# Ignalina/znippy

Measured on NVIDIA B200. Metric: decode+blake3-verify GB/s (device), higher is better.
Workload: dtype u8/u32

## Files before the change

znippy_b200/csrc/blake3_kernels.cuh:

```cuda
#pragma once
#include "blake3.cuh"
#include "xxh_verify.cuh"

namespace zn {

ZN_D const uint8_t* content_ptr(const BlobDesc& d, const uint8_t* blobs_base, const uint8_t* out_base) {
  return (d.flags & F_COMPRESSED) ? out_base + d.dst_off : blobs_base + d.src_off;
}

constexpr int kB3Warps = 8;
constexpr int kB3RowBytes = 128;
constexpr int kB3RowStride = kB3RowBytes + 16;
constexpr int kB3Stages = 2;
constexpr int kB3StageBytes = 32 * kB3RowStride;
constexpr int kB3SmemPerWarp = kB3Stages * kB3StageBytes;
constexpr int kB3RowsPerIssue = 32 / (kB3RowBytes / 16);

ZN_D void cp_async16(void* smem_dst, const void* gmem_src) {
  const uint32_t s = (uint32_t)__cvta_generic_to_shared(smem_dst);
  asm volatile("cp.async.cg.shared.global [%0], [%1], 16;\n" ::"r"(s), "l"(gmem_src) : "memory");
}
ZN_D void cp_async_commit() { asm volatile("cp.async.commit_group;\n" ::: "memory"); }
template <int N>
ZN_D void cp_async_wait() { asm volatile("cp.async.wait_group %0;\n" ::"n"(N) : "memory"); }
// ... 87 lines not shown

__global__ void __launch_bounds__(kB3Warps * 32) k_b3_chunks(const BlobDesc* __restrict__ blobs,
                                                              const uint32_t* __restrict__ chunk_prefix,
                                                              uint32_t n_blobs, uint32_t chunk_lo, uint32_t chunk_hi,
                                                              const uint8_t* __restrict__ blobs_base,
                                                              const uint8_t* __restrict__ out_base,
                                                              uint32_t* cvs, uint32_t one) {
  extern __shared__ __align__(16) uint8_t b3_smem[];
  const uint32_t lane = threadIdx.x & 31u, warp = threadIdx.x >> 5;
  uint8_t* wbuf = b3_smem + warp * kB3SmemPerWarp;
  const uint32_t n_tiles = (chunk_hi - chunk_lo + 31u) >> 5;
  const uint32_t warps_total = gridDim.x * kB3Warps;
  for (uint32_t tile = blockIdx.x * kB3Warps + warp; tile < n_tiles; tile += warps_total) {
    const uint32_t g = chunk_lo + tile * 32u + lane;
    const bool act = g < chunk_hi;
    const uint8_t* ptr = nullptr;
    uint32_t len = 0, ctr = 0;
    bool root = false, skip = false;
    if (act) {
      uint32_t lo = 0, hi = n_blobs;
      while (hi - lo > 1) {
        const uint32_t mid = (lo + hi) >> 1;
        if (__ldg(chunk_prefix + mid) <= g) lo = mid; else hi = mid;
      }
      const BlobDesc d = blobs[lo];
      skip = (d.flags & F_HASHED) != 0;
      ctr = g - __ldg(chunk_prefix + lo);
      ptr = content_ptr(d, blobs_base, out_base) + (uint64_t)ctr * kChunk;
      const uint64_t remain = d.dst_cap - (uint64_t)ctr * kChunk;
      len = remain < kChunk ? (uint32_t)remain : kChunk;
      root = d.n_chunks == 1;
    }
    if (__all_sync(0xFFFFFFFFu, !act || skip)) continue;
    uint32_t cv[8];
    b3_warp_tile(wbuf, ptr, len, ctr, root, act && !skip, lane, one, cv);
    if (act && !skip) b3::store_cv(cvs + (uint64_t)g * 8, cv);
  }
}

ZN_D void finish_blob(const BlobDesc& d, uint32_t blob, const uint32_t (&cv)[8], uint32_t* __restrict__ digests,
                      const uint32_t* __restrict__ expect, uint32_t* __restrict__ status, const uint8_t* blobs_base,
                      const uint8_t* out_base) {
  b3::store_cv(digests + (uint64_t)blob * 8, cv);
  if (out_base && status[blob] == S_OK && xxh_row_bad(d, blobs_base, out_base)) status[blob] = S_DECODE_ERROR;
  if ((d.flags & F_HAS_EXPECT) && status[blob] == S_OK) {
    bool eq = true;
#pragma unroll
    for (int i = 0; i < 8; i++) eq &= (__ldg(expect + (uint64_t)blob * 8 + i) == cv[i]);
    if (!eq) status[blob] = S_DIGEST_MISMATCH;
  }
}

__global__ void __launch_bounds__(128) k_b3_tree_small(const BlobDesc* __restrict__ blobs,
                                                       const uint32_t* __restrict__ list, uint32_t n_list,
                                                       uint32_t* cvs, uint32_t* __restrict__ digests,
                                                       const uint32_t* __restrict__ expect,
                                                       uint32_t* __restrict__ status, uint32_t one,
                                                       const uint8_t* blobs_base, const uint8_t* out_base) {
  const uint32_t t = blockIdx.x * blockDim.x + threadIdx.x;
  if (t >= n_list) return;
  const uint32_t blob = list[t];
  const BlobDesc d = blobs[blob];
  uint32_t* base = cvs + d.cv_base * 8;
  uint32_t n = d.n_chunks;
  uint32_t l[8], r[8], o[8];
  while (n > 1) {
    const uint32_t pairs = n >> 1;
    for (uint32_t j = 0; j < pairs; j++) {
      b3::load_cv(base + (uint64_t)(2 * j) * 8, l);
      b3::load_cv(base + (uint64_t)(2 * j + 1) * 8, r);
      b3::parent(l, r, n == 2, o, one);
      b3::store_cv(base + (uint64_t)j * 8, o);
    }
    if (n & 1) {
      b3::load_cv(base + (uint64_t)(n - 1) * 8, l);
      b3::store_cv(base + (uint64_t)pairs * 8, l);
    }
    n = pairs + (n & 1);
  }
  b3::load_cv(base, o);
  finish_blob(d, blob, o, digests, expect, status, blobs_base, out_base);
}

__global__ void __launch_bounds__(512) k_b3_tree_large(const BlobDesc* __restrict__ blobs,
                                                       const uint32_t* __restrict__ list,
                                                       uint32_t* cvs, uint32_t* cvs2, uint32_t* __restrict__ digests,
                                                       const uint32_t* __restrict__ expect,
                                                       uint32_t* __restrict__ status, uint32_t one,
                                                       const uint8_t* blobs_base, const uint8_t* out_base) {
  const uint32_t blob = list[blockIdx.x];
  const BlobDesc d = blobs[blob];
  uint32_t* src = cvs + d.cv_base * 8;
  uint32_t* dst = cvs2 + d.cv_base * 8;
  uint32_t n = d.n_chunks;
  uint32_t l[8], r[8], o[8];
  while (n > 1) {
    const uint32_t pairs = n >> 1, items = pairs + (n & 1);
    for (uint32_t j = threadIdx.x; j < items; j += blockDim.x) {
      b3::load_cv(src + (uint64_t)(2 * j) * 8, l);
      if (j < pairs) {
        b3::load_cv(src + (uint64_t)(2 * j + 1) * 8, r);
        b3::parent(l, r, n == 2, o, one);
      } else {
#pragma unroll
        for (int i = 0; i < 8; i++) o[i] = l[i];
      }
      b3::store_cv(dst + (uint64_t)j * 8, o);
    }
    __syncthreads();
    uint32_t* t = src; src = dst; dst = t;
    n = items;
  }
  if (threadIdx.x == 0) {
    b3::load_cv(src, o);
    finish_blob(d, blob, o, digests, expect, status, blobs_base, out_base);
  }
}

constexpr uint32_t kTreeSmallMax = 64;

}
```

znippy_b200/csrc/fused_ws.cuh:

```cuda
#pragma once
#include "blake3_kernels.cuh"
#include "decode_kernels.cuh"

namespace zn {

constexpr int kWsTeamThreads = 128;
constexpr int kWsTeams = 2;
constexpr int kWsTeamWarps = kWsTeamThreads / 32;
constexpr int kWsDecWarps = kWsTeams * kWsTeamWarps;
constexpr int kWsHashWarps = 16;
constexpr int kWsThreads = 32 * (kWsDecWarps + kWsHashWarps);
constexpr uint32_t kWsTileBytes = 32u * kChunk;

struct WsDecRegion {
  alignas(128) uint8_t tile[kTileBytes];
  alignas(16) uint8_t src[kSrcStage + 32];
  DecShared sh;
  uint32_t base;
};

constexpr uint32_t kWsTeamBytes =
    ((sizeof(WsDecRegion) > (size_t)kWsTeamWarps * kB3SmemPerWarp ? sizeof(WsDecRegion) : (size_t)kWsTeamWarps * kB3SmemPerWarp) + 127u) & ~127u;
constexpr uint32_t kWsSmemBytes = kWsTeams * kWsTeamBytes + kWsHashWarps * kB3SmemPerWarp;
static_assert(kWsSmemBytes <= 227u * 1024u, "one CTA per SM");

struct WsQueue {
  uint32_t* ctl;
  unsigned long long* ent;
  uint32_t total;
};

#ifdef ZN_WS_DEBUG
__device__ unsigned long long g_ws_dbg[4];
ZN_D unsigned long long ws_now() { unsigned long long t; asm volatile("mov.u64 %0, %%globaltimer;" : "=l"(t)); return t; }
#endif

ZN_D void ws_push(const WsQueue& q, uint32_t list_idx, uint32_t first_tile, uint32_t count) {
  if (!count) return;
  __threadfence();
  const uint32_t pos = atomicAdd(q.ctl + 1, count);
  for (uint32_t i = 0; i < count; i++)
    *reinterpret_cast<volatile unsigned long long*>(q.ent + pos + i) = ((unsigned long long)list_idx << 32) | (first_tile + i + 1u);
}

struct WsHook {
  WsQueue q;
  uint32_t list_idx, cap, pushed;
  ZN_D void after_block(const Team& t, zs::ExecState& es) {
    if (es.pos - es.wm >= (1u << 20)) zs::mem_sync(t, es);
    const uint32_t w = es.wm < cap ? es.wm : cap;
    const uint32_t ready = w / kWsTileBytes;
    if (t.tid == t.n - 1u && ready > pushed) ws_push(q, list_idx, pushed, ready - pushed);
    if (ready > pushed) pushed = ready;
  }
  ZN_D void finish(const Team&, zs::ExecState&) {}
};

__global__ void __launch_bounds__(kWsThreads, 1)
    k_decode_ws(const BlobDesc* __restrict__ blobs, const uint32_t* __restrict__ list, uint32_t n_list, const uint8_t* blobs_base,
                uint8_t* out_base, uint8_t* lit_scratch, uint32_t* status, uint32_t* produced, uint32_t* work_counter, uint32_t* cvs,
                WsQueue q, uint32_t one) {
  extern __shared__ __align__(128) uint8_t ws_smem[];
  const uint32_t warp = threadIdx.x >> 5, lane = threadIdx.x & 31u;
#ifdef ZN_WS_DEBUG
  if (threadIdx.x == 0) atomicMin(&g_ws_dbg[0], ws_now());
#endif

  if (warp < (uint32_t)kWsDecWarps) {
    const uint32_t team = warp / kWsTeamWarps;
    WsDecRegion* dr = reinterpret_cast<WsDecRegion*>(ws_smem + team * kWsTeamBytes);
    const Team t{threadIdx.x - team * kWsTeamThreads, (uint32_t)kWsTeamThreads, 1u + team};
    DecShared* sh = &dr->sh;
    if (t.tid == 0) sh->tile = dr->tile;
    zs::init_luts(t, sh);
    uint8_t* lit = lit_scratch + (size_t)(blockIdx.x * kWsTeams + team) * kLitStride;
    uint32_t predef = 0;
    for (;;) {
      if (t.tid == 0) dr->base = atomicAdd(work_counter, 1u);
      team_sync(t);
      const uint32_t base = dr->base;
      if (base >= n_list) break;
      const uint32_t blob = list[base];
      const BlobDesc d = blobs[blob];
      WsHook hook{q, base, (uint32_t)d.dst_cap, 0u};
      uint32_t st, got = 0;
      if (d.src_len >= 0xFFFFFFF0ull || d.dst_cap >= 0xFFFFFFF0ull) {
        st = S_UNSUPPORTED;
      } else {
        const uint8_t* src = blobs_base + d.src_off;
        if (d.src_len <= kSrcStage) {
          team_copy(t, dr->src + 16, src, (uint32_t)d.src_len);
          team_sync(t);
          src = dr->src + 16;
        }
        if (d.flags & F_LZ4_BLOCK) {
          st = decode_lz4_block(t, sh, src, (uint32_t)d.src_len, out_base + d.dst_off, (uint32_t)d.dst_cap, &got);
        } else {
          st = decode_blob(t, sh, src, (uint32_t)d.src_len, out_base + d.dst_off, (uint32_t)d.dst_cap, lit, predef, &got, hook);
        }
        if (st == S_OK && got != (uint32_t)d.dst_cap) st = S_SIZE_MISMATCH;
      }
      if (t.tid < kBulkIssuers) bulk_wait_all();
      team_sync(t);
      if (t.tid == 0) {
        status[blob] = st;
        produced[blob] = got;
      }
      if (t.tid == t.n - 1u) {
        const uint32_t n_tiles = (d.n_chunks + 31u) / 32u;
        ws_push(q, base, hook.pushed, n_tiles - hook.pushed);
      }
    }
#ifdef ZN_WS_DEBUG
    if (t.tid == 0) { atomicMax(&g_ws_dbg[1], ws_now()); atomicMax(&g_ws_dbg[3], (unsigned long long)*(volatile uint32_t*)q.ctl); }
#endif
    team_sync(t);
  }

  uint8_t* wbuf = warp < (uint32_t)kWsDecWarps
                      ? ws_smem + (warp / kWsTeamWarps) * kWsTeamBytes + (warp % kWsTeamWarps) * kB3SmemPerWarp
                      : ws_smem + kWsTeams * kWsTeamBytes + (warp - kWsDecWarps) * kB3SmemPerWarp;
  for (;;) {
    uint32_t idx = 0, e_lo = 0, e_hi = 0;
    if (lane == 0) {
      idx = atomicAdd(q.ctl, 1u);
      if (idx < q.total) {
        unsigned long long e;
        uint32_t spins = 0;
        while ((e = *reinterpret_cast<volatile unsigned long long*>(q.ent + idx)) == 0ull) {
          __nanosleep(100);
          if (++spins > (1u << 25) || ((spins & 4095u) == 0 && *reinterpret_cast<volatile uint32_t*>(q.ctl + 2))) {
            atomicExch(q.ctl + 2, 1u);
            idx = 0xFFFFFFFFu;
            break;
          }
        }
        __threadfence();
        e_lo = (uint32_t)e;
        e_hi = (uint32_t)(e >> 32);
      }
    }
    idx = __shfl_sync(0xFFFFFFFFu, idx, 0);
    if (idx >= q.total) break;
    const uint32_t tile = __shfl_sync(0xFFFFFFFFu, e_lo, 0) - 1u, li = __shfl_sync(0xFFFFFFFFu, e_hi, 0);
    const BlobDesc d = blobs[list[li]];
    const uint32_t cap = (uint32_t)d.dst_cap;
    const uint32_t g = tile * 32u + lane;
    const bool act = g < d.n_chunks;
    const uint32_t rem = act ? cap - min(cap, g * kChunk) : 0u;
    uint32_t cv[8];
#ifdef ZN_WS_NOHASH
    for (int k = 0; k < 8; k++) cv[k] = 0;
#else
    b3_warp_tile(wbuf, out_base + d.dst_off + (size_t)g * kChunk, rem < kChunk ? rem : kChunk, g, d.n_chunks == 1, act, lane, one, cv);
#endif
    if (act) b3::store_cv(cvs + (size_t)d.cv_base * 8 + (size_t)g * 8, cv);
  }
#ifdef ZN_WS_DEBUG
  if (lane == 0) atomicMax(&g_ws_dbg[2], ws_now());
#endif
}

}
```

znippy_b200/csrc/znippy_cuda.cu:

```cuda
#include <cuda_runtime.h>

#include <algorithm>
#include <chrono>
#include <cstdio>
#include <cstring>
#include <mutex>
#include <numeric>
#include <string>
#include <unordered_map>
#include <vector>

#define ZN_BACKBITS_DEPTH 1
#include "../../include/znippy_cuda.h"
#include "blake3_kernels.cuh"
#include "host_api.h"
#include "decode_kernels.cuh"
#include "par_kernel.cuh"
#include "fused_ws.cuh"

using namespace zn;

struct zn_ctx {
  int device = 0;
  int sm_count = 0;
  cudaStream_t stream = nullptr;
  cudaStream_t stream2 = nullptr;
  void* pinned = nullptr;
  size_t pinned_bytes = 0;
  uint8_t* plan_pin = nullptr;
  size_t plan_pin_cap = 0, plan_pin_used = 0;
  template <typename T>
  T* arena(size_t count) {
    plan_pin_used = (plan_pin_used + 63) & ~(size_t)63;
    T* r = reinterpret_cast<T*>(plan_pin + plan_pin_used);
    plan_pin_used += count * sizeof(T);
    return r;
  }
  uint8_t* d_lit = nullptr;
  uint8_t* d_par = nullptr;
  uint32_t dec_grid = 0;
  uint32_t dec_grid_small = 0;
  uint8_t* d_in = nullptr;
  size_t d_in_cap = 0;
  uint8_t* d_out = nullptr;
  size_t d_out_cap = 0;
  CompressScratch cs;
  struct ZScratch {
    zp::ZBlock* blocks = nullptr; uint32_t* comp_list = nullptr; size_t slots = 0;
    zp::FseD* tabs = nullptr; size_t tab_sets = 0;
    zp::SeqRec16* recs = nullptr; size_t seqs = 0;
    zp::SeqP1* p1 = nullptr; size_t p1s = 0;
    uint8_t* lits = nullptr; size_t lit16 = 0;
    zp::ZPools* pools = nullptr;
  } zs;
  uint64_t launches = 0;
  std::string err;
};

enum PlanKind { PLAN_DECODE_VERIFY = 1, PLAN_HASH = 2, PLAN_COMPRESS = 3 };

enum DecClass {
  DC_PIPE = 0,
  DC_BIGPAT,
  DC_BIGRAW,
  DC_SMALL,
  DC_MID,
  DC_COUNT
};

struct zn_plan {
  zn_ctx* ctx = nullptr;
  int kind = 0;
  uint32_t n = 0;
  uint32_t total_chunks = 0;
  uint32_t n_dec = 0, n_small = 0, n_large = 0, n_pieces = 0;
  BlobDesc* d_blobs = nullptr;
  uint32_t* d_chunk_prefix = nullptr;
  uint32_t *d_list_dec = nullptr, *d_list_small = nullptr, *d_list_large = nullptr;
  uint32_t *d_piece_blob = nullptr, *d_piece_idx = nullptr;
  uint64_t* d_magic_off = nullptr;
  uint32_t n_magic = 0;
  uint32_t *d_cvs = nullptr, *d_digests = nullptr, *d_expect = nullptr, *d_status = nullptr, *d_produced = nullptr,
           *d_counter = nullptr, *d_wsq = nullptr, *d_cvs2 = nullptr, *d_status0 = nullptr;
  uint32_t ws_tiles = 0;
  bool ran_ws = false;
  cudaEvent_t ev[4] = {nullptr, nullptr, nullptr, nullptr};
  cudaStream_t last_stream = nullptr;
  bool ran = false;
  uint32_t cls_off[DC_COUNT + 1] = {0};
  uint32_t n_hashed = 0;
  zp::ZBlob* d_zb = nullptr;
  uint32_t nzb = 0;
  size_t z_slots = 0, z_tabs = 0, z_seqs = 0, z_lit16 = 0;
  uint64_t z_mean = 0;
  bool uploads_synced = false;
  uint32_t launches_per_run = 0;
  CompressScratch cs;
  CompressPrep cp;
  zn_plan* hp = nullptr;
  bool envelope = false;
  uint64_t capacity = 0;
  std::vector<uint32_t> h_status;
};

static const int kDecodeThreads = 128;
static const int kDecodeCtasPerSm = 4;

#define ZN_CUDA(ctx, call)                                                              \
  do {                                                                                  \
    cudaError_t e__ = (call);                                                           \
    if (e__ != cudaSuccess) {                                                           \
      (ctx)->err = std::string(#call) + ": " + cudaGetErrorString(e__);                 \
      return ZN_E_CUDA;                                                                 \
    }                                                                                   \
  } while (0)

extern "C" int zn_abi_version(void) { return ZN_ABI_VERSION; }

extern "C" int zn_device_count(void) {
  int n = 0;
  if (cudaGetDeviceCount(&n) != cudaSuccess) return 0;
  return n;
}

extern "C" const char* zn_strerror(int code) {
  switch (code) {
    case ZN_OK: return "ok";
    case ZN_E_ARG: return "invalid argument";
    case ZN_E_CUDA: return "CUDA error";
    case ZN_E_NOMEM: return "out of memory";
    case ZN_E_STATE: return "call out of order";
    default: return "unknown error";
  }
}

extern "C" const char* zn_status_name(uint32_t s) {
  switch (s) {
    case ZN_S_OK: return "OK";
    case ZN_S_DECODE_ERROR: return "DECODE_ERROR";
    case ZN_S_DIGEST_MISMATCH: return "DIGEST_MISMATCH";
    case ZN_S_DST_TOO_SMALL: return "DST_TOO_SMALL";
    case ZN_S_UNSUPPORTED: return "UNSUPPORTED";
    case ZN_S_SIZE_MISMATCH: return "SIZE_MISMATCH";
    default: return "?";
  }
}

static void build_predef(PredefTables* p) {
  static zs::FseTable t;
  uint16_t next[64];
  zs::fse_build(&t, zs::kLLDefault, 36, 6, next);
  for (int i = 0; i < 64; i++) p->ll[i] = t.e[i];
  zs::fse_build(&t, zs::kOFDefault, 29, 5, next);
  for (int i = 0; i < 32; i++) p->of[i] = t.e[i];
  zs::fse_build(&t, zs::kMLDefault, 53, 6, next);
  for (int i = 0; i < 64; i++) p->ml[i] = t.e[i];
}

extern "C" zn_ctx* zn_ctx_create(int device, size_t staging_bytes) {
  int ndev = 0;
  if (cudaGetDeviceCount(&ndev) != cudaSuccess || device < 0 || device >= ndev) return nullptr;
  if (cudaSetDevice(device) != cudaSuccess) return nullptr;
  zn_ctx* c = new zn_ctx();
  c->device = device;
  cudaDeviceProp prop;
  if (cudaGetDeviceProperties(&prop, device) != cudaSuccess) { delete c; return nullptr; }
// ... 164 lines not shown
    BlobDesc& d = descs[i];
    const bool comp = kind == PLAN_DECODE_VERIFY && compressed && compressed[i];
    d.src_off = src_off[i];
    d.src_len = src_len[i];
    if (comp && compressed[i] == 3) {
      if (d.src_off < 4) { delete p; c->err = "compressed == 3 needs four bytes in front of the payload"; return nullptr; }
      d.src_off -= 4;
      d.src_len += 4;
      magic_off.push_back(d.src_off);
    }
    d.dst_off = out_off ? out_off[i] : 0;
    d.dst_cap = kind == PLAN_DECODE_VERIFY ? (out_len ? out_len[i] : 0) : src_len[i];
    bool skip = false;
    if (!comp && kind == PLAN_DECODE_VERIFY && d.dst_cap != d.src_len) {
      status0[i] = S_SIZE_MISMATCH;
      any_status = true;
      skip = true;
      d.src_len = 0;
      d.dst_cap = 0;
    }
    const uint64_t nc = std::max<uint64_t>(1, (d.dst_cap + kChunk - 1) / kChunk);
    d.n_chunks = (uint32_t)nc;
    d.cv_base = chunks;
    d.flags = (comp ? F_COMPRESSED : 0u) | (expect && !skip ? F_HAS_EXPECT : 0u) | (comp && compressed[i] == 2 ? F_LZ4_BLOCK : 0u);
    prefix[i] = (uint32_t)chunks;
    chunks += nc;
    if (chunks > 0xFFFFFFF0ull) { delete p; c->err = "batch too large (chunk count)"; return nullptr; }
    if (comp) {
      const bool big = d.dst_cap >= (512u << 10), pat = d.src_len * 64 <= d.dst_cap, lz4b = (d.flags & F_LZ4_BLOCK) != 0;
      int k;
      if (big && pat && !lz4b) k = DC_BIGPAT;
      else if (!lz4b && !pat && d.src_len < d.dst_cap && d.dst_cap >= 4096 && d.dst_cap < 0xFFFFFFF0ull) k = DC_PIPE;
      else if (big) k = DC_BIGRAW;
      else if (d.dst_cap <= (64u << 10)) k = DC_SMALL;
      else k = DC_MID;
      cls[k].push_back(i);
    } else if (gather_raw && kind == PLAN_DECODE_VERIFY && !skip)
      for (uint64_t o = 0, k = 0; o < d.dst_cap; o += kGatherPiece, k++) { pblob.push_back(i); pidx.push_back((uint32_t)k); }
    if (nc <= kTreeSmallMax) lsmall_a[n_lsmall++] = i; else llarge.push_back(i);
  }
  prefix[n] = (uint32_t)chunks;
  p->total_chunks = (uint32_t)chunks;
  uint32_t* ldec = c->arena<uint32_t>(n);
  uint32_t n_ldec = 0;
  for (int k = 0; k < DC_COUNT; k++) {
    auto& L = cls[k];
    bool sorted_desc = true;
    for (size_t j = 1; j < L.size() && sorted_desc; j++) sorted_desc = descs[L[j]].dst_cap <= descs[L[j - 1]].dst_cap;
    if (!sorted_desc) std::stable_sort(L.begin(), L.end(), [&](uint32_t x, uint32_t y) { return descs[x].dst_cap > descs[y].dst_cap; });
    p->cls_off[k] = n_ldec;
    if (!L.empty()) memcpy(ldec + n_ldec, L.data(), L.size() * 4);
    n_ldec += (uint32_t)L.size();
  }
  p->cls_off[DC_COUNT] = n_ldec;
  p->n_dec = n_ldec;
  for (uint32_t i : cls[DC_BIGPAT]) { descs[i].flags |= F_HASHED; p->ws_tiles += (descs[i].n_chunks + 31u) / 32u; p->n_hashed++; }
  std::vector<zp::ZBlob> zb(cls[DC_PIPE].size());
  {
    uint64_t slots = 0, seqs = 0, lit16 = 0, tabs = 0, bytes = 0;
    for (size_t j = 0; j < zb.size(); j++) {
      const uint64_t cap = descs[cls[DC_PIPE][j]].dst_cap;
      const uint32_t sc = (uint32_t)(cap / 16384 + 8);
      memset(&zb[j], 0, sizeof zb[j]);
      zb[j].blob = cls[DC_PIPE][j];
      zb[j].slot0 = (uint32_t)slots;
      zb[j].slot_cap = sc;
      slots += sc;
      seqs += cap / 5 + 64;
      lit16 += cap / 16 + 2ull * sc + 2;
      tabs += cap / 32768 + 2;
      bytes += cap;
    }
    const uint64_t lim = 0xFFFFFFF0ull;
    p->nzb = (uint32_t)zb.size();
    p->z_slots = (size_t)std::min(slots, lim);
    p->z_seqs = (size_t)std::min(seqs, lim);
    p->z_lit16 = (size_t)std::min(lit16, lim);
    p->z_tabs = (size_t)std::min(tabs, lim);
    p->z_mean = zb.empty() ? 0 : bytes / zb.size();
    if (slots > lim) { delete p; c->err = "batch too large (zstd block slots)"; return nullptr; }
  }
  p->n_small = n_lsmall;
  p->n_large = (uint32_t)llarge.size();
  p->n_pieces = (uint32_t)pblob.size();
  p->n_magic = (uint32_t)magic_off.size();
  bool ok = upload(c, &p->d_blobs, descs, n) && upload(c, &p->d_chunk_prefix, prefix, (size_t)n + 1) &&
            upload(c, &p->d_list_dec, ldec, n_ldec) && upload(c, &p->d_list_small, lsmall_a, n_lsmall) &&
            upload(c, &p->d_list_large, llarge.data(), llarge.size()) &&
            upload(c, &p->d_piece_blob, pblob.data(), pblob.size()) && upload(c, &p->d_piece_idx, pidx.data(), pidx.size()) &&
            upload(c, &p->d_magic_off, magic_off.data(), magic_off.size()) &&
            upload(c, &p->d_expect, (const uint32_t*)expect, expect ? (size_t)n * 8 : 0) &&
            upload(c, &p->d_cvs, (const uint32_t*)nullptr, (size_t)chunks * 8) &&
            upload(c, &p->d_cvs2, (const uint32_t*)nullptr, llarge.empty() ? 0 : (size_t)chunks * 8) &&
            upload(c, &p->d_digests, (const uint32_t*)nullptr, (size_t)n * 8) &&
            upload(c, &p->d_status, (const uint32_t*)nullptr, n) && upload(c, &p->d_produced, (const uint32_t*)nullptr, n) &&
            upload(c, &p->d_counter, (const uint32_t*)nullptr, 16) &&
            upload(c, &p->d_wsq, (const uint32_t*)nullptr, cls[DC_BIGPAT].empty() ? 0 : 6 + 2 * (size_t)p->ws_tiles) &&
            upload(c, &p->d_zb, zb.data(), zb.size());
  if (ok && any_status) ok = upload(c, &p->d_status0, status0, n);
  for (int i = 0; ok && i < 4; i++) ok = cudaEventCreate(&p->ev[i]) == cudaSuccess;
  if (ok) ok = cudaStreamSynchronize(c->stream) == cudaSuccess;
  if (!ok) {
    c->err = std::string("plan allocation failed: ") + cudaGetErrorString(cudaGetLastError());
    zn_plan_destroy(p);
    return nullptr;
  }
  p->uploads_synced = true;
  return p;
}

extern "C" zn_plan* zn_plan_decode_verify(zn_ctx* ctx, uint32_t n, const uint64_t* h_blob_off, const uint64_t* h_blob_len,
                                          const uint8_t* h_compressed, const uint64_t* h_out_off,
                                          const uint64_t* h_out_len, const uint8_t* h_expect_digest) {
  if (n && (!h_out_len || !h_compressed)) return nullptr;
  return plan_build(ctx, PLAN_DECODE_VERIFY, n, h_blob_off, h_blob_len, h_compressed, h_out_off, h_out_len,
                    h_expect_digest, h_out_off != nullptr);
}

extern "C" zn_plan* zn_plan_hash(zn_ctx* ctx, uint32_t n, const uint64_t* h_off, const uint64_t* h_len,
                                 const uint8_t* h_expect_digest) {
  return plan_build(ctx, PLAN_HASH, n, h_off, h_len, nullptr, nullptr, nullptr, h_expect_digest, false);
}

extern "C" int zn_plan_fused(const zn_plan* p) { return p && p->cls_off[DC_BIGPAT + 1] > p->cls_off[DC_BIGPAT] ? 1 : 0; }

extern "C" int zn_plan_class_counts(const zn_plan* p, uint32_t counts[5]) {
  if (!p || !counts) return ZN_E_ARG;
  if (p->kind == PLAN_COMPRESS) return ZN_E_STATE;
  for (int k = 0; k < DC_COUNT; k++) counts[k] = p->cls_off[k + 1] - p->cls_off[k];
  return ZN_OK;
}

extern "C" int zn_plan_pipeline_fallbacks(zn_plan* p, uint32_t* rows) {
  if (!p || !rows) return ZN_E_ARG;
  if (p->kind == PLAN_COMPRESS) return ZN_E_STATE;
  *rows = 0;
  if (!p->nzb || !p->ran) return ZN_OK;
  cudaSetDevice(p->ctx->device);
  if (cudaStreamSynchronize(p->last_stream) != cudaSuccess) { p->ctx->err = cudaGetErrorString(cudaGetLastError()); return ZN_E_CUDA; }
  std::vector<zp::ZBlob> hz(p->nzb);
  if (cudaMemcpy(hz.data(), p->d_zb, sizeof(zp::ZBlob) * p->nzb, cudaMemcpyDeviceToHost) != cudaSuccess) { p->ctx->err = cudaGetErrorString(cudaGetLastError()); return ZN_E_CUDA; }
  for (auto& b : hz) *rows += b.state != 0;
  return ZN_OK;
}

extern "C" void zn_plan_destroy(zn_plan* p) {
  if (!p) return;
  cudaSetDevice(p->ctx->device);
  if (p->ran) cudaStreamSynchronize(p->last_stream);
  void* ptrs[] = {p->d_blobs, p->d_chunk_prefix, p->d_list_dec, p->d_list_small, p->d_list_large, p->d_piece_blob,
                  p->d_piece_idx, p->d_cvs, p->d_digests, p->d_expect, p->d_status, p->d_produced, p->d_counter, p->d_wsq, p->d_cvs2,
                  p->d_zb, p->d_status0, p->d_magic_off};
  for (void* q : ptrs)
    if (q) cudaFreeAsync(q, p->ctx->stream);
  for (auto& e : p->ev)
    if (e) cudaEventDestroy(e);
  if (p->hp) zn_plan_destroy(p->hp);
  p->cs.release();
  delete p;
}

template <typename T>
static bool zgrow(T** ptr, size_t* have, size_t want, size_t bytes_per) {
  if (*have >= want) return true;
  if (*ptr) cudaFree(*ptr);
  *ptr = nullptr;
  *have = 0;
  const size_t cap = want + want / 8 + 16;
  if (cudaMalloc((void**)ptr, cap * bytes_per) != cudaSuccess) { cudaGetLastError(); return false; }
  *have = cap;
  return true;
}

static int run_pipeline(zn_plan* p, const uint8_t* d_blobs, uint8_t* d_out, cudaStream_t st, uint32_t* launches) {
  zn_ctx* c = p->ctx;
  auto& z = c->zs;
  if (!z.pools && cudaMalloc((void**)&z.pools, sizeof(zp::ZPools)) != cudaSuccess) { c->err = "zstd pipeline scratch allocation failed"; cudaGetLastError(); return ZN_E_NOMEM; }
  {
    const size_t slots_before = z.slots;
    size_t dummy = slots_before;
    if (!zgrow(&z.blocks, &z.slots, p->z_slots, sizeof(zp::ZBlock)) || !zgrow(&z.comp_list, &dummy, p->z_slots, 4) ||
        !zgrow(&z.tabs, &z.tab_sets, p->z_tabs, sizeof(zp::FseD) * zp::kTabSet) || !zgrow(&z.recs, &z.seqs, p->z_seqs, sizeof(zp::SeqRec16)) || !zgrow(&z.p1, &z.p1s, p->z_seqs, sizeof(zp::SeqP1)) ||
        !zgrow(&z.lits, &z.lit16, p->z_lit16 + 4, 16)) {
      c->err = "zstd pipeline scratch allocation failed";
      return ZN_E_NOMEM;
    }
  }
  zp::ZArgs a;
  a.blobs = p->d_blobs; a.blobs_base = d_blobs; a.zb = p->d_zb; a.nzb = p->nzb; a.blocks = z.blocks; a.pools = z.pools;
  a.comp_list = z.comp_list; a.tabs = z.tabs; a.recs = z.recs; a.lits = z.lits; a.p1 = z.p1;
  const bool prof = getenv("ZN_ZPROF") != nullptr;
  cudaEvent_t pe[9];
  if (prof) for (auto& e : pe) cudaEventCreate(&e);
  uint32_t* ctr = p->d_counter + DC_COUNT;
  zp::PipelineLaunch L;
  L.a = a;
  L.slots = (uint32_t)p->z_slots; L.seq_cap = (uint32_t)p->z_seqs; L.lit_cap16 = (uint32_t)p->z_lit16; L.tab_cap = (uint32_t)p->z_tabs;
  L.sm_count = (uint32_t)c->sm_count;
  L.mean_bytes = p->z_mean;
  L.d_out = d_out; L.produced = p->d_produced; L.exec_counter = ctr;
  const uint32_t pipe_launches = zp::pipeline_enqueue(L, st, prof ? pe : nullptr);
  const uint32_t* list = p->d_list_dec + p->cls_off[DC_PIPE];
  const uint32_t grid = std::min<uint32_t>(p->nzb, c->dec_grid);
  k_decode<kDecodeThreads, 1><<<grid, kDecodeThreads, 0, st>>>(p->d_blobs, list, p->nzb, d_blobs, d_out, c->d_lit, p->d_status,
                                                            p->d_produced, ctr + 1, nullptr, 1u, &p->d_zb[0].state,
                                                            (uint32_t)(sizeof(zp::ZBlob) / 4));
  if (prof) {
    cudaEventRecord(pe[7], st);
    cudaEventSynchronize(pe[7]);
    static const char* names[] = {"walk", "tables", "seq", "lit", "chain", "exec", "legacy"};
    zp::ZPools hp;
    cudaMemcpy(&hp, z.pools, sizeof hp, cudaMemcpyDeviceToHost);
    std::vector<zp::ZBlob> hz(p->nzb);
    cudaMemcpy(hz.data(), p->d_zb, sizeof(zp::ZBlob) * p->nzb, cudaMemcpyDeviceToHost);
    uint32_t handed = 0;
    for (auto& b : hz) handed += b.state != 0;
    fprintf(stderr, "zpipe: %u blobs (%u handed back), %u blocks, %u seqs, %u table sets, %u lit16 |", p->nzb, handed, hp.comp_used, hp.seq_used, hp.tab_used, hp.lit_used16);
    for (int i = 0; i < 7; i++) { float ms = 0; cudaEventElapsedTime(&ms, pe[i], pe[i + 1]); fprintf(stderr, " %s %.3f", names[i], ms); }
    if (getenv("ZN_ZPROF_SEQ1")) { float ms = 0; if (cudaEventElapsedTime(&ms, pe[2], pe[8]) == cudaSuccess) fprintf(stderr, " (seq phase 1 %.3f)", ms); else cudaGetLastError(); }
    fprintf(stderr, " ms\n");
    zp::pipeline_trace_dump();
    for (auto& e : pe) cudaEventDestroy(e);
  }
  *launches += pipe_launches + 1;
  return ZN_OK;
}

extern "C" int zn_plan_run(zn_plan* p, const uint8_t* d_blobs, uint8_t* d_out, void* stream_v) {
  if (!p) return ZN_E_ARG;
  if (p->kind == PLAN_COMPRESS) return ZN_E_STATE;
  zn_ctx* c = p->ctx;
  cudaSetDevice(c->device);
  cudaStream_t st = stream_v ? (cudaStream_t)stream_v : c->stream;
  if (p->n && !d_blobs) return ZN_E_ARG;
  if (p->n_dec && !d_out) return ZN_E_ARG;
  if (st != c->stream && !p->uploads_synced) {
    ZN_CUDA(c, cudaStreamSynchronize(c->stream));
    p->uploads_synced = true;
  }
  uint32_t launches = 0;
  ZN_CUDA(c, cudaEventRecord(p->ev[0], st));
  if (p->n) {
    if (p->d_status0) ZN_CUDA(c, cudaMemcpyAsync(p->d_status, p->d_status0, (size_t)p->n * 4, cudaMemcpyDeviceToDevice, st));
    else ZN_CUDA(c, cudaMemsetAsync(p->d_status, 0, (size_t)p->n * 4, st));
    ZN_CUDA(c, cudaMemsetAsync(p->d_counter, 0, 4 * 16, st));
  }
  if (p->n_magic) {
    k_patch_magic<<<(p->n_magic + 255) / 256, 256, 0, st>>>(const_cast<uint8_t*>(d_blobs), p->d_magic_off, p->n_magic);
    launches++;
  }
  if (p->n_pieces && d_out) {
    const uint32_t grid = std::min<uint32_t>(p->n_pieces, (uint32_t)c->sm_count * 16u);
    k_gather_raw<<<grid, 256, 0, st>>>(p->d_blobs, p->d_piece_blob, p->d_piece_idx, p->n_pieces, d_blobs, d_out);
    launches++;
  }
  auto cls_n = [&](int k) { return p->cls_off[k + 1] - p->cls_off[k]; };
  auto cls_list = [&](int k) { return p->d_list_dec + p->cls_off[k]; };
  if (p->nzb) {
    const int rc = run_pipeline(p, d_blobs, d_out, st, &launches);
    if (rc != ZN_OK) return rc;
  }
  if (const uint32_t nd = cls_n(DC_BIGPAT)) {
    ZN_CUDA(c, cudaMemsetAsync(p->d_wsq, 0, 24 + 8 * (size_t)p->ws_tiles, st));
    p->ran_ws = true;
    const uint32_t phantom = getenv("ZN_WS_TEST_STALL") ? 1u : 0u;
    WsQueue q{p->d_wsq, reinterpret_cast<unsigned long long*>(p->d_wsq + 4), p->ws_tiles + phantom};
    uint32_t wgrid = (uint32_t)c->sm_count;
    if (const char* gs = getenv("ZN_WS_GRID")) wgrid = std::max(1, std::min<int>((int)wgrid, atoi(gs)));
    k_decode_ws<<<wgrid, kWsThreads, kWsSmemBytes, st>>>(p->d_blobs, cls_list(DC_BIGPAT), nd, d_blobs, d_out, c->d_lit, p->d_status,
                                                         p->d_produced, p->d_counter + DC_BIGPAT, p->d_cvs, q, 1u);
    launches++;
  }
  if (const uint32_t nd = cls_n(DC_BIGRAW)) {
    const uint32_t max_grid = (uint32_t)c->sm_count;
    if (!c->d_par && cudaMalloc(&c->d_par, (size_t)max_grid * par::kParScratchPerCta) != cudaSuccess) {
      c->err = "block-parallel decode scratch allocation failed";
      cudaGetLastError();
      return ZN_E_NOMEM;
    }
    par::k_decode_par<<<std::min<uint32_t>(nd, max_grid), par::kParThreads, sizeof(par::ParShared), st>>>(
        p->d_blobs, cls_list(DC_BIGRAW), nd, d_blobs, d_out, c->d_par, p->d_status, p->d_produced, p->d_counter + DC_BIGRAW);
    launches++;
  }
  if (const uint32_t nd = cls_n(DC_SMALL)) {
    const uint32_t grid = std::min<uint32_t>((nd + 1) / 2, c->dec_grid_small);
    k_decode<32, 2><<<grid, 32, 0, st>>>(p->d_blobs, cls_list(DC_SMALL), nd, d_blobs, d_out, c->d_lit, p->d_status, p->d_produced,
                                         p->d_counter + DC_SMALL, nullptr, 1u, nullptr, 0u);
    launches++;
  }
  if (const uint32_t nd = cls_n(DC_MID)) {
    const uint32_t grid = std::min<uint32_t>((nd + 3) / 4, c->dec_grid);
    k_decode<kDecodeThreads, 4><<<grid, kDecodeThreads, 0, st>>>(p->d_blobs, cls_list(DC_MID), nd, d_blobs, d_out, c->d_lit,
                                                              p->d_status, p->d_produced, p->d_counter + DC_MID, nullptr, 1u,
                                                              nullptr, 0u);
    launches++;
  }
  ZN_CUDA(c, cudaEventRecord(p->ev[1], st));
  if (p->total_chunks && p->n_hashed != p->n) {
    const uint32_t tiles = (p->total_chunks + 31u) / 32u;
    const uint32_t ctas = (tiles + kB3Warps - 1) / kB3Warps;
    const uint32_t grid = std::min<uint32_t>(ctas, (uint32_t)c->sm_count * 3u);
    k_b3_chunks<<<grid, kB3Warps * 32, kB3Warps * kB3SmemPerWarp, st>>>(p->d_blobs, p->d_chunk_prefix, p->n, 0u, p->total_chunks,
                                                                       d_blobs, d_out, p->d_cvs, 1u);
    launches++;
  }
  ZN_CUDA(c, cudaEventRecord(p->ev[2], st));
  const uint8_t* xxh_out = p->n_dec ? d_out : nullptr;
  if (p->n_small) {
    k_b3_tree_small<<<(p->n_small + 127) / 128, 128, 0, st>>>(p->d_blobs, p->d_list_small, p->n_small, p->d_cvs, p->d_digests,
                                                              p->d_expect, p->d_status, 1u, d_blobs, xxh_out);
    launches++;
  }
  if (p->n_large) {
    k_b3_tree_large<<<p->n_large, 512, 0, st>>>(p->d_blobs, p->d_list_large, p->d_cvs, p->d_cvs2, p->d_digests, p->d_expect, p->d_status, 1u,
                                                d_blobs, xxh_out);
    launches++;
  }
  ZN_CUDA(c, cudaEventRecord(p->ev[3], st));
  ZN_CUDA(c, cudaGetLastError());
  p->launches_per_run = launches;
  c->launches += launches;
  p->last_stream = st;
  p->ran = true;
  return ZN_OK;
}

extern "C" int zn_plan_results(zn_plan* p, uint32_t* h_status, uint8_t* h_digests) {
  if (!p) return ZN_E_ARG;
  if (!p->ran) return ZN_E_STATE;
  zn_ctx* c = p->ctx;
  cudaSetDevice(c->device);
  if (p->kind == PLAN_COMPRESS) {
    ZN_CUDA(c, cudaStreamSynchronize(p->last_stream));
    if (h_status && p->n) memcpy(h_status, p->h_status.data(), (size_t)p->n * 4);
    return h_digests && p->hp ? zn_plan_results(p->hp, nullptr, h_digests) : ZN_OK;
  }
  if (h_status && p->n) ZN_CUDA(c, cudaMemcpyAsync(h_status, p->d_status, (size_t)p->n * 4, cudaMemcpyDeviceToHost, p->last_stream));
  if (h_digests && p->n) ZN_CUDA(c, cudaMemcpyAsync(h_digests, p->d_digests, (size_t)p->n * 32, cudaMemcpyDeviceToHost, p->last_stream));
  uint32_t stall = 0;
  if (p->d_wsq && p->ran_ws) ZN_CUDA(c, cudaMemcpyAsync(&stall, p->d_wsq + 2, 4, cudaMemcpyDeviceToHost, p->last_stream));
  ZN_CUDA(c, cudaStreamSynchronize(p->last_stream));
  if (stall) { c->err = "fused decode+hash kernel stalled (internal error): results are incomplete"; return ZN_E_CUDA; }
  return ZN_OK;
}

extern "C" uint32_t zn_plan_launches(const zn_plan* p) { return p ? p->launches_per_run : 0; }

extern "C" int zn_plan_last_ms(zn_plan* p, float ms[4]) {
  if (!p || !ms) return ZN_E_ARG;
  if (!p->ran) return ZN_E_STATE;
  zn_ctx* c = p->ctx;
  cudaSetDevice(c->device);
  ZN_CUDA(c, cudaEventSynchronize(p->ev[3]));
  ZN_CUDA(c, cudaEventElapsedTime(&ms[0], p->ev[0], p->ev[3]));
  ZN_CUDA(c, cudaEventElapsedTime(&ms[1], p->ev[0], p->ev[1]));
  ZN_CUDA(c, cudaEventElapsedTime(&ms[2], p->ev[1], p->ev[2]));
  ZN_CUDA(c, cudaEventElapsedTime(&ms[3], p->ev[2], p->ev[3]));
  return ZN_OK;
}

extern "C" zn_plan* zn_plan_compress(zn_ctx* c, uint32_t n, const uint64_t* h_src_off, const uint64_t* h_src_len, int level,
                                     int codec, int digests) {
  if (!c) return nullptr;
  const int base = codec & ~ZN_CODEC_ENVELOPE;
  if (base != ZN_CODEC_ZSTD && base != ZN_CODEC_LZ4) {
    c->err = "zn_plan_compress: codec must be ZN_CODEC_ZSTD or ZN_CODEC_LZ4, optionally | ZN_CODEC_ENVELOPE";
    return nullptr;
  }
  if (n && (!h_src_off || !h_src_len)) { c->err = "zn_plan_compress: null size arrays"; return nullptr; }
  cudaSetDevice(c->device);
  zn_plan* p = new zn_plan();
  p->ctx = c;
  p->kind = PLAN_COMPRESS;
  p->n = n;
  p->envelope = (codec & ZN_CODEC_ENVELOPE) != 0;
  p->h_status.assign(n, 0);
  for (uint32_t i = 0; i < n; i++) {
    uint8_t hdr[ZN_ENVELOPE_ZNB1_MAX_HEADER];
    p->capacity += p->envelope ? zn_envelope_znb1_header(ZN_PAYLOAD_RAW, h_src_len[i], hdr, sizeof hdr) + h_src_len[i]
                               : compress_bound(h_src_len[i], base);
  }
  std::string err;
  if (compress_prepare(&p->cs, c->stream, c->sm_count, h_src_off, h_src_len, n, level, base, nullptr, &p->cp, p->h_status.data(),
                       &err) != 0) {
    c->err = "zn_plan_compress: " + err;
    zn_plan_destroy(p);
    return nullptr;
  }
  if (digests && n && !(p->hp = zn_plan_hash(c, n, h_src_off, h_src_len, nullptr))) {
    zn_plan_destroy(p);
    return nullptr;
  }
  bool ok = true;
  for (int i = 0; ok && i < 4; i++) ok = cudaEventCreate(&p->ev[i]) == cudaSuccess;
  if (ok) ok = cudaStreamSynchronize(c->stream) == cudaSuccess;
  if (!ok) {
    c->err = std::string("zn_plan_compress: ") + cudaGetErrorString(cudaGetLastError());
    zn_plan_destroy(p);
// ... 499 lines not shown
          if (r <= 0) { io_err = 1; return; }
          done += (uint64_t)r;
        }
      });
    });
  };
  auto start_write = [&](Batch& B) {
    B.writer = std::thread([&B, &io_err, out_fd, uncompressed_size, fdata_offset, io_threads, out_root, paths, path_off]() {
      parallel_rows(B.n, io_threads, [&](uint32_t i) {
        const uint32_t s = B.status[i];
        const bool ok = s == ZN_S_OK || s == ZN_S_DIGEST_MISMATCH;
        int fd = out_fd[B.a + i];
        const bool lazy = fd == -2 && out_root && paths && path_off;
        if (lazy) {
          std::string full(out_root);
          full += '/';
          full.append(paths + path_off[B.a + i], (size_t)(path_off[B.a + i + 1] - path_off[B.a + i]));
          fd = open(full.c_str(), O_CREAT | O_WRONLY | O_TRUNC, 0644);
          if (fd < 0) { io_err = 1; return; }
        }
        if (ok && fd >= 0) {
          uint64_t done = 0, len = uncompressed_size[B.a + i];
          while (done < len) {
            const ssize_t r = pwrite(fd, B.pin_out.p + B.out_off[i] + done, len - done, (off_t)(fdata_offset[B.a + i] + done));
            if (r <= 0) { io_err = 1; break; }
            done += (uint64_t)r;
          }
        }
        if (lazy) close(fd);
      });
    });
  };
  int rc = ZN_OK;
  uint64_t next = row_lo;
  int cur = 0;
  bool have = false;
  if (next < row_hi) {
    if (!claim(bt[0], next)) { c->err = "pinned staging allocation failed"; return ZN_E_NOMEM; }
    next = bt[0].b;
    start_read(bt[0]);
    have = true;
  }
  while (have && rc == ZN_OK) {
    Batch& B = bt[cur];
    Batch& O = bt[cur ^ 1];
    join(B.reader);
    if (io_err) { c->err = "failed to read blob from archive"; rc = ZN_E_ARG; break; }
    bool more = false;
    if (next < row_hi) {
      join(O.writer);
      if (io_err) { c->err = "pwrite to output file failed"; rc = ZN_E_ARG; break; }
      if (!claim(O, next)) { c->err = "pinned staging allocation failed"; rc = ZN_E_NOMEM; break; }
      next = O.b;
      start_read(O);
      more = true;
    }
    rc = zn_decode_verify_batch(c, B.pin_in.p, B.in_off.data(), blob_size + B.a, compressed + B.a, uncompressed_size + B.a,
                                checksums + 32 * B.a, out_fd ? B.pin_out.p : nullptr, out_fd ? B.out_off.data() : nullptr, B.n,
                                B.status.data(), nullptr);
    if (rc != ZN_OK) break;
    for (uint32_t i = 0; i < B.n; i++) {
      stats->total_chunks++;
      const uint32_t s = B.status[i];
      if (s != ZN_S_OK && s != ZN_S_DIGEST_MISMATCH) { stats->decode_errors++; continue; }
      const uint64_t len = uncompressed_size[B.a + i];
      stats->total_written_bytes += len;
      if (s == ZN_S_OK) stats->verified_bytes += len;
      else {
        stats->corrupt_bytes += len;
        if (corrupt_rows_out) corrupt_rows_out[stats->corrupt_rows] = B.a + i;
        stats->corrupt_rows++;
      }
    }
    if (out_fd) start_write(B);
    have = more;
    cur ^= 1;
  }
  for (auto& B : bt) { join(B.reader); join(B.writer); }
  if (rc == ZN_OK && io_err) { c->err = "pwrite to output file failed"; rc = ZN_E_ARG; }
  return rc;
}

#ifdef ZN_WS_DEBUG
extern "C" void zn_debug_ws_times(unsigned long long* out, int reset) {
  if (reset) {
    unsigned long long init[4] = {~0ull, 0, 0, 0};
    cudaMemcpyToSymbol(g_ws_dbg, init, sizeof init);
  } else {
    cudaDeviceSynchronize();
    cudaMemcpyFromSymbol(out, g_ws_dbg, 32);
  }
}
#endif
```

Before: 1838.

## Split large-blob BLAKE3 tree reduction across multiple CTAs per blob

The large-blob Merkle tree reduction previously ran one 512-thread CTA per blob, which leaves most SMs idle when there are only a few large blobs. Each blob is now split into 1024-chunk subtrees, each reduced by its own 128-thread CTA. The last CTA to finish, detected through an atomic counter per row, then reduces the subtree roots. CV loads switch to L2-only __ldcg so results written by other CTAs are read correctly. This adds a host-built work list, a counter reset, and extra debug instrumentation that only compiles under a flag.

After: 1823, median of 6. Within noise of the previous version (-0.8%).

```diff
diff --git a/znippy_b200/csrc/blake3_kernels.cuh b/znippy_b200/csrc/blake3_kernels.cuh
--- a/znippy_b200/csrc/blake3_kernels.cuh
+++ b/znippy_b200/csrc/blake3_kernels.cuh
@@ -193,37 +193,74 @@
   finish_blob(d, blob, o, digests, expect, status, blobs_base, out_base);
 }
 
-__global__ void __launch_bounds__(512) k_b3_tree_large(const BlobDesc* __restrict__ blobs,
-                                                       const uint32_t* __restrict__ list,
-                                                       uint32_t* cvs, uint32_t* cvs2, uint32_t* __restrict__ digests,
-                                                       const uint32_t* __restrict__ expect,
-                                                       uint32_t* __restrict__ status, uint32_t one,
-                                                       const uint8_t* blobs_base, const uint8_t* out_base) {
-  const uint32_t blob = list[blockIdx.x];
-  const BlobDesc d = blobs[blob];
-  uint32_t* src = cvs + d.cv_base * 8;
-  uint32_t* dst = cvs2 + d.cv_base * 8;
-  uint32_t n = d.n_chunks;
+constexpr uint32_t kTreeSub = 1024;
+constexpr int kTreeThreads = 128;
+
+ZN_D void load_cv_cg(const uint32_t* p, uint32_t (&cv)[8]) {
+  const uint4 a = __ldcg(reinterpret_cast<const uint4*>(p)), b = __ldcg(reinterpret_cast<const uint4*>(p + 4));
+  cv[0] = a.x; cv[1] = a.y; cv[2] = a.z; cv[3] = a.w; cv[4] = b.x; cv[5] = b.y; cv[6] = b.z; cv[7] = b.w;
+}
+
+ZN_D const uint32_t* b3_tree_reduce(const uint32_t* src, uint32_t stride, uint32_t* a, uint32_t* b, uint32_t n, bool root,
+                                    uint32_t one) {
   uint32_t l[8], r[8], o[8];
   while (n > 1) {
     const uint32_t pairs = n >> 1, items = pairs + (n & 1);
     for (uint32_t j = threadIdx.x; j < items; j += blockDim.x) {
-      b3::load_cv(src + (uint64_t)(2 * j) * 8, l);
+      load_cv_cg(src + (uint64_t)(2 * j) * stride * 8, l);
       if (j < pairs) {
-        b3::load_cv(src + (uint64_t)(2 * j + 1) * 8, r);
-        b3::parent(l, r, n == 2, o, one);
+        load_cv_cg(src + (uint64_t)(2 * j + 1) * stride * 8, r);
+        b3::parent(l, r, root && n == 2, o, one);
       } else {
 #pragma unroll
         for (int i = 0; i < 8; i++) o[i] = l[i];
       }
-      b3::store_cv(dst + (uint64_t)j * 8, o);
+      b3::store_cv(a + (uint64_t)j * 8, o);
     }
     __syncthreads();
-    uint32_t* t = src; src = dst; dst = t;
+    src = a;
+    stride = 1;
+    a = b;
+    b = const_cast<uint32_t*>(src);
     n = items;
   }
+  return src;
+}
+
+__global__ void __launch_bounds__(kTreeThreads) k_b3_tree_large(const BlobDesc* __restrict__ blobs,
+                                                                const uint32_t* __restrict__ list,
+                                                                const uint32_t* __restrict__ work, uint32_t* row_done,
+                                                                uint32_t* cvs, uint32_t* cvs2, uint32_t* __restrict__ digests,
+                                                                const uint32_t* __restrict__ expect,
+                                                                uint32_t* __restrict__ status, uint32_t one,
+                                                                const uint8_t* blobs_base, const uint8_t* out_base) {
+  __shared__ uint32_t s_last;
+  const uint32_t li = work[2 * blockIdx.x], sub = work[2 * blockIdx.x + 1];
+  const uint32_t blob = list[li];
+  const BlobDesc d = blobs[blob];
+  const uint32_t n_sub = (d.n_chunks + kTreeSub - 1) / kTreeSub;
+  uint32_t* row = cvs + (uint64_t)d.cv_base * 8;
+  uint32_t* mine = row + (uint64_t)sub * kTreeSub * 8;
+  const uint32_t n = min(kTreeSub, d.n_chunks - sub * kTreeSub);
+  const uint32_t* res = b3_tree_reduce(mine, 1, cvs2 + ((uint64_t)d.cv_base + (uint64_t)sub * kTreeSub) * 8, mine, n, n_sub == 1, one);
+  uint32_t o[8];
+  if (n_sub > 1) {
+    if (threadIdx.x == 0) {
+      if (res != mine) {
+        load_cv_cg(res, o);
+        b3::store_cv(mine, o);
+      }
+      __threadfence();
+      s_last = atomicAdd(row_done + li, 1u) == n_sub - 1u;
+    }
+    __syncthreads();
+    if (!s_last) return;
+    __threadfence();
+    if (threadIdx.x == 0) row_done[li] = 0;
+    res = b3_tree_reduce(row, kTreeSub, cvs2 + (uint64_t)d.cv_base * 8, row, n_sub, true, one);
+  }
   if (threadIdx.x == 0) {
-    b3::load_cv(src, o);
+    load_cv_cg(res, o);
     finish_blob(d, blob, o, digests, expect, status, blobs_base, out_base);
   }
 }
diff --git a/znippy_b200/csrc/fused_ws.cuh b/znippy_b200/csrc/fused_ws.cuh
--- a/znippy_b200/csrc/fused_ws.cuh
+++ b/znippy_b200/csrc/fused_ws.cuh
@@ -31,8 +31,11 @@
 };
 
 #ifdef ZN_WS_DEBUG
-__device__ unsigned long long g_ws_dbg[4];
+constexpr int kWsDbgWords = 16 + 192;
+__device__ unsigned long long g_ws_dbg[kWsDbgWords];
 ZN_D unsigned long long ws_now() { unsigned long long t; asm volatile("mov.u64 %0, %%globaltimer;" : "=l"(t)); return t; }
+ZN_D unsigned long long ws_warpbit() { uint32_t w; asm volatile("mov.u32 %0, %%warpid;" : "=r"(w)); return 1ull << (w & 63u); }
+ZN_D uint32_t ws_smid() { uint32_t s; asm volatile("mov.u32 %0, %%smid;" : "=r"(s)); return s; }
 #endif
 
 ZN_D void ws_push(const WsQueue& q, uint32_t list_idx, uint32_t first_tile, uint32_t count) {
@@ -46,7 +49,17 @@
 struct WsHook {
   WsQueue q;
   uint32_t list_idx, cap, pushed;
+#ifdef ZN_WS_DEBUG
+  unsigned long long t_prev = ws_now();
+#endif
   ZN_D void after_block(const Team& t, zs::ExecState& es) {
+#ifdef ZN_WS_DEBUG
+    if (t.tid == 0) {
+      const unsigned long long now = ws_now(), dt = now - t_prev;
+      t_prev = now;
+      atomicAdd(&g_ws_dbg[4], dt); atomicAdd(&g_ws_dbg[5], 1ull); atomicMax(&g_ws_dbg[6], dt);
+    }
+#endif
     if (es.pos - es.wm >= (1u << 20)) zs::mem_sync(t, es);
     const uint32_t w = es.wm < cap ? es.wm : cap;
     const uint32_t ready = w / kWsTileBytes;
@@ -63,13 +76,21 @@
   extern __shared__ __align__(128) uint8_t ws_smem[];
   const uint32_t warp = threadIdx.x >> 5, lane = threadIdx.x & 31u;
 #ifdef ZN_WS_DEBUG
-  if (threadIdx.x == 0) atomicMin(&g_ws_dbg[0], ws_now());
+  if (threadIdx.x == 0) {
+    const unsigned long long now = ws_now();
+    atomicMin(&g_ws_dbg[0], now);
+    if (blockIdx.x == 0) { g_ws_dbg[10] = clock64(); g_ws_dbg[11] = now; }
+  }
 #endif
 
   if (warp < (uint32_t)kWsDecWarps) {
     const uint32_t team = warp / kWsTeamWarps;
     WsDecRegion* dr = reinterpret_cast<WsDecRegion*>(ws_smem + team * kWsTeamBytes);
     const Team t{threadIdx.x - team * kWsTeamThreads, (uint32_t)kWsTeamThreads, 1u + team};
+#ifdef ZN_WS_DEBUG
+    if (t.tid == 0) atomicOr(&g_ws_dbg[7 + team], ws_warpbit());
+    if (t.tid == t.n - 1u) atomicOr(&g_ws_dbg[9], ws_warpbit());
+#endif
     DecShared* sh = &dr->sh;
     if (t.tid == 0) sh->tile = dr->tile;
     zs::init_luts(t, sh);
@@ -127,6 +148,9 @@
       if (idx < q.total) {
         unsigned long long e;
         uint32_t spins = 0;
+#ifdef ZN_WS_DEBUG
+        const long long w0 = clock64();
+#endif
         while ((e = *reinterpret_cast<volatile unsigned long long*>(q.ent + idx)) == 0ull) {
           __nanosleep(100);
           if (++spins > (1u << 25) || ((spins & 4095u) == 0 && *reinterpret_cast<volatile uint32_t*>(q.ctl + 2))) {
@@ -135,6 +159,9 @@
             break;
           }
         }
+#ifdef ZN_WS_DEBUG
+        if (spins) atomicAdd(&g_ws_dbg[16 + ws_smid() % 192u], (unsigned long long)(clock64() - w0));
+#endif
         __threadfence();
         e_lo = (uint32_t)e;
         e_hi = (uint32_t)(e >> 32);
@@ -157,7 +184,11 @@
     if (act) b3::store_cv(cvs + (size_t)d.cv_base * 8 + (size_t)g * 8, cv);
   }
 #ifdef ZN_WS_DEBUG
-  if (lane == 0) atomicMax(&g_ws_dbg[2], ws_now());
+  if (lane == 0) {
+    const unsigned long long now = ws_now();
+    atomicMax(&g_ws_dbg[2], now);
+    if (blockIdx.x == 0 && atomicMax(&g_ws_dbg[13], now) < now) g_ws_dbg[12] = clock64();
+  }
 #endif
 }
 
diff --git a/znippy_b200/csrc/znippy_cuda.cu b/znippy_b200/csrc/znippy_cuda.cu
--- a/znippy_b200/csrc/znippy_cuda.cu
+++ b/znippy_b200/csrc/znippy_cuda.cu
@@ -73,7 +73,7 @@
   int kind = 0;
   uint32_t n = 0;
   uint32_t total_chunks = 0;
-  uint32_t n_dec = 0, n_small = 0, n_large = 0, n_pieces = 0;
+  uint32_t n_dec = 0, n_small = 0, n_large = 0, n_pieces = 0, n_tree = 0;
   BlobDesc* d_blobs = nullptr;
   uint32_t* d_chunk_prefix = nullptr;
   uint32_t *d_list_dec = nullptr, *d_list_small = nullptr, *d_list_large = nullptr;
@@ -82,6 +82,7 @@
   uint32_t n_magic = 0;
   uint32_t *d_cvs = nullptr, *d_digests = nullptr, *d_expect = nullptr, *d_status = nullptr, *d_produced = nullptr,
            *d_counter = nullptr, *d_wsq = nullptr, *d_cvs2 = nullptr, *d_status0 = nullptr;
+  uint32_t* d_tree = nullptr;
   uint32_t ws_tiles = 0;
   bool ran_ws = false;
   cudaEvent_t ev[4] = {nullptr, nullptr, nullptr, nullptr};
@@ -412,11 +413,16 @@
   }
   p->n_small = n_lsmall;
   p->n_large = (uint32_t)llarge.size();
+  std::vector<uint32_t> tree;
+  for (uint32_t j = 0; j < p->n_large; j++)
+    for (uint32_t s = 0; s * kTreeSub < descs[llarge[j]].n_chunks; s++) { tree.push_back(j); tree.push_back(s); }
+  p->n_tree = (uint32_t)(tree.size() / 2);
+  tree.resize(tree.size() + p->n_large, 0u);
   p->n_pieces = (uint32_t)pblob.size();
   p->n_magic = (uint32_t)magic_off.size();
   bool ok = upload(c, &p->d_blobs, descs, n) && upload(c, &p->d_chunk_prefix, prefix, (size_t)n + 1) &&
             upload(c, &p->d_list_dec, ldec, n_ldec) && upload(c, &p->d_list_small, lsmall_a, n_lsmall) &&
-            upload(c, &p->d_list_large, llarge.data(), llarge.size()) &&
+            upload(c, &p->d_list_large, llarge.data(), llarge.size()) && upload(c, &p->d_tree, tree.data(), tree.size()) &&
             upload(c, &p->d_piece_blob, pblob.data(), pblob.size()) && upload(c, &p->d_piece_idx, pidx.data(), pidx.size()) &&
             upload(c, &p->d_magic_off, magic_off.data(), magic_off.size()) &&
             upload(c, &p->d_expect, (const uint32_t*)expect, expect ? (size_t)n * 8 : 0) &&
@@ -480,7 +486,7 @@
   if (p->ran) cudaStreamSynchronize(p->last_stream);
   void* ptrs[] = {p->d_blobs, p->d_chunk_prefix, p->d_list_dec, p->d_list_small, p->d_list_large, p->d_piece_blob,
                   p->d_piece_idx, p->d_cvs, p->d_digests, p->d_expect, p->d_status, p->d_produced, p->d_counter, p->d_wsq, p->d_cvs2,
-                  p->d_zb, p->d_status0, p->d_magic_off};
+                  p->d_zb, p->d_status0, p->d_magic_off, p->d_tree};
   for (void* q : ptrs)
     if (q) cudaFreeAsync(q, p->ctx->stream);
   for (auto& e : p->ev)
@@ -642,8 +648,8 @@
     launches++;
   }
   if (p->n_large) {
-    k_b3_tree_large<<<p->n_large, 512, 0, st>>>(p->d_blobs, p->d_list_large, p->d_cvs, p->d_cvs2, p->d_digests, p->d_expect, p->d_status, 1u,
-                                                d_blobs, xxh_out);
+    k_b3_tree_large<<<p->n_tree, kTreeThreads, 0, st>>>(p->d_blobs, p->d_list_large, p->d_tree, p->d_tree + 2 * (size_t)p->n_tree,
+                                                        p->d_cvs, p->d_cvs2, p->d_digests, p->d_expect, p->d_status, 1u, d_blobs, xxh_out);
     launches++;
   }
   ZN_CUDA(c, cudaEventRecord(p->ev[3], st));
@@ -1309,13 +1315,14 @@
 }
 
 #ifdef ZN_WS_DEBUG
+extern "C" int zn_debug_ws_words() { return kWsDbgWords; }
 extern "C" void zn_debug_ws_times(unsigned long long* out, int reset) {
   if (reset) {
-    unsigned long long init[4] = {~0ull, 0, 0, 0};
+    unsigned long long init[kWsDbgWords] = {~0ull};
     cudaMemcpyToSymbol(g_ws_dbg, init, sizeof init);
   } else {
     cudaDeviceSynchronize();
-    cudaMemcpyFromSymbol(out, g_ws_dbg, 32);
+    cudaMemcpyFromSymbol(out, g_ws_dbg, sizeof(unsigned long long) * kWsDbgWords);
   }
 }
 #endif
```
